# georgesterpu/avsr-tf1

Measured on AMD Instinct MI355X. Metric: utterances/sec (train step) at B=64 T_a=500 T_v=75, higher is better.
Workload: dtype f32; 1 GPU; c4: AV dual-attention (bimodal) video 1x256 + audio 3x256 uni-LSTM, scaled_luong, B=64 T_a=500x80 T_v=75 L=40; utterances_per_gpu=64, global_batch=64, T_a=500, F_a=80, T_v=75, F_v=128, T_dec=40, parallelism=dp1, video_frontend=resnet_cnn, launch=hipgraph, dropout=True

## Files before the change

### avsr-tf1_amd/csrc/rnn_persist.hip

```cpp
#include "step.h"
#include "avsr_hip.h"
#include "prof.h"
#include "persist.h"

#define P_MAX_TASKS 8
#define P_MAXC 8

namespace avsr {

struct PTask {
  const float* wt; const float* bias; const int* len;
  float* gates; float* cs;
  float* out; long out_sb, out_st;
  float* hs_w; long hs_sb, hs_st;
  const float* hs_r; long hsr_sb, hsr_st;
  const float* x_r; long x_sb, x_st;
  float* xt_w; long xt_sb, xt_st;
  float* h_final; float* c_final;
  int* done; const int* done_lower;
  int B, T, H, in, hoisted, reverse, nct, nct_lower, wg_begin, nrt, uw, part, prio;
  const int32_t* seed; float k_st, k_out, k_in; uint32_t r_st, r_out, r_in; int in_W, in_coff;
};
struct PLaunch { int ntask, wpx, ngroups, b0, npart, pwg[2]; int* err; int* claim; PTask task[P_MAX_TASKS]; };

__device__ __forceinline__ bool wait_ge2(const int* c0, int n0, const int* c1, int n1, int* err) {
  for (int spins = 0; spins < (1 << 21); ++spins) {
    const int a = c0 ? __hip_atomic_load(c0, __ATOMIC_RELAXED, __HIP_MEMORY_SCOPE_AGENT) : n0;
    const int b = c1 ? __hip_atomic_load(c1, __ATOMIC_RELAXED, __HIP_MEMORY_SCOPE_AGENT) : n1;
    if (a >= n0 && b >= n1) return true;
    if ((spins & 1023) == 1023 && __hip_atomic_load(err, __ATOMIC_RELAXED, __HIP_MEMORY_SCOPE_AGENT)) return false;
    __builtin_amdgcn_s_sleep(1);
  }
  __hip_atomic_store(err, 1, __ATOMIC_RELAXED, __HIP_MEMORY_SCOPE_AGENT);
  return false;
}

#ifdef PERSIST_TIMING
#define TICK(k) { const long now_ = __builtin_amdgcn_s_memtime(); tm[k] += now_ - last_; last_ = now_; }
#else
#define TICK(k)
#endif
#define P_XC 4
#define P_HC 4

__global__ __launch_bounds__(256) void rnn_persist_fwd_kernel(const PLaunch L) {
  __shared__ __attribute__((aligned(16))) float red[4][2][16][16];
  int ti = 0;
#pragma unroll
  for (int i = 1; i < P_MAX_TASKS; ++i)
    if (i < L.ntask && (int)blockIdx.x >= L.task[i].wg_begin) ti = i;
  ti = __builtin_amdgcn_readfirstlane(ti);
  const PTask& tk = L.task[ti];
  const int local = blockIdx.x - tk.wg_begin;
  const int rt = local / tk.nct, ct = local % tk.nct;
  const int row0 = rt * 16, col0 = ct * 32, unit0 = ct * 8;
  const int tid = threadIdx.x, lane = tid & 63, wave = tid >> 6;
  const int i = lane & 15, q = lane >> 4;
  const int H = tk.H, T = tk.T;
  const int hoisted = tk.hoisted, reverse = tk.reverse;
  const int Kx = hoisted ? 0 : tk.in;
  const int ncx = (Kx + 15) >> 4, nchh = (H + 15) >> 4;
  const int xg0 = (wave * ncx) / 4, nxw = ((wave + 1) * ncx) / 4 - xg0;
  const int hg0 = (wave * nchh) / 4, nhw = ((wave + 1) * nchh) / 4 - hg0;
  const long ldw = tk.in + H;

  f32x4 wx[P_XC][2], wh[P_HC][2];
#pragma unroll
  for (int nt = 0; nt < 2; ++nt) {
    const int col = col0 + nt * 16 + i;
#pragma unroll
    for (int c = 0; c < P_XC; ++c) {
      const int k = (xg0 + c) * 16 + 4 * q;
      wx[c][nt] = (c < nxw && col < 4 * H && k < Kx) ? ld4(tk.wt + (long)col * ldw + k) : f32x4{0.f, 0.f, 0.f, 0.f};
    }
#pragma unroll
    for (int c = 0; c < P_HC; ++c) {
      const int k = (hg0 + c) * 16 + 4 * q;
      wh[c][nt] = (c < nhw && col < 4 * H && k < H) ? ld4(tk.wt + (long)col * ldw + tk.in + k) : f32x4{0.f, 0.f, 0.f, 0.f};
    }
  }

  const int er = tid >> 3, eu = tid & 7;
  const int b = row0 + er, u = unit0 + eu;
  const bool eok = tid < 128 && b < tk.B && u < H;
  const int len_b = eok ? (tk.len ? tk.len[b] : T) : 0;
  f32x4 bias4 = {0.f, 0.f, 0.f, 0.f};
  if (eok && tk.bias) bias4 = ld4(tk.bias + u * 4);
  float c_state = 0.f, h_state = 0.f;

  const int ab = row0 + i;
  const bool aok = ab < tk.B;
  const int len_a = aok ? (tk.len ? tk.len[ab] : T) : 0;
  const int xrow = (int)(ab * tk.x_sb) + 4 * q, hrow = (int)(ab * tk.hsr_sb) + 4 * q;
  const int x_st = (int)tk.x_st, h_st = (int)tk.hsr_st;
  const float* const x_r = tk.x_r; const float* const hs_r = tk.hs_r;
  const int nct = tk.nct, nct_lower = tk.nct_lower;
  int* const done_mine = tk.done + (long)rt * T;
  const int* const done_low = hoisted ? nullptr : tk.done_lower + (long)rt * T;
  const int rec_b = b * T * H + u;
  const int out_b = (int)(b * tk.out_sb) + u, hsw_b = (int)(b * tk.hs_sb) + u, xtw_b = (int)(b * tk.xt_sb) + u;
  const int out_st = (int)tk.out_st, hs_st = (int)tk.hs_st, xt_st = (int)tk.xt_st;
  float* const gates_p = tk.gates; float* const cs_p = tk.cs; float* const out_p = tk.out;
  float* const hsw_p = tk.hs_w; float* const xtw_p = tk.xt_w;
  const bool drop_on = tk.seed != nullptr;
  const uint32_t seedv = drop_on ? (uint32_t)tk.seed[0] : 0u;
  const float k_st = tk.k_st, k_out = tk.k_out, k_in = tk.k_in;
  const uint32_t r_st = tk.r_st, r_out = tk.r_out, r_in = tk.r_in;
  const int in_W = tk.in_W, in_coff = tk.in_coff;

  f32x4 xcur[P_XC];
#pragma unroll
  for (int c = 0; c < P_XC; ++c) xcur[c] = f32x4{0.f, 0.f, 0.f, 0.f};
  auto load_x = [&](int t, f32x4* dst) {
    const bool v = aok && t < len_a;
    const int xo = xrow + (reverse ? len_a - 1 - t : t) * x_st;
#pragma unroll
    for (int c = 0; c < P_XC; ++c) {
      const int k = (xg0 + c) * 16;
      dst[c] = (c < nxw && v && k + 4 * q < Kx) ? ld4_sc1(x_r + (xo + k)) : f32x4{0.f, 0.f, 0.f, 0.f};
    }
  };
  if (done_low) {
    if (tid == 0) wait_ge2(done_low, nct_lower, nullptr, 0, L.err);
    __syncthreads();
    load_x(0, xcur);
  }

  f32x4 znext = {0.f, 0.f, 0.f, 0.f};
  if (eok && hoisted && 0 < len_b) znext = ld4(gates_p + (long)(rec_b + (reverse ? len_b - 1 : 0) * H) * 4);
#ifdef PERSIST_TIMING
  long tm[6] = {0, 0, 0, 0, 0, 0};
#endif
  for (int t = 0; t < T; ++t) {
#ifdef PERSIST_TIMING
    long last_ = __builtin_amdgcn_s_memtime();
#endif
    f32x4 zpre = znext;
    asm volatile("" : "+v"(zpre));
    if (tid == 0) {
      const int tl = t + 1 < T ? t + 1 : T - 1;
      wait_ge2(t > 0 ? done_mine + (t - 1) : nullptr, nct, done_low ? done_low + tl : nullptr, nct_lower, L.err);
    }
    lds_barrier();
    TICK(0)

    const bool avalid = aok && t < len_a;
    const int ho_ = hrow + (reverse ? len_a - 1 - t : t) * h_st;
    f32x4 hv[P_HC];
#pragma unroll
    for (int c = 0; c < P_HC; ++c) {
      const int k = (hg0 + c) * 16;
      hv[c] = (c < nhw && avalid && t > 0 && k + 4 * q < H) ? ld4_sc1(hs_r + (ho_ + k)) : f32x4{0.f, 0.f, 0.f, 0.f};
    }
    f32x4 acc[2][2];
#pragma unroll
    for (int nt = 0; nt < 2; ++nt)
#pragma unroll
      for (int e = 0; e < 2; ++e) acc[nt][e] = f32x4{0.f, 0.f, 0.f, 0.f};
#pragma unroll
    for (int c = 0; c < P_XC; ++c)
      if (c < nxw) {
#pragma unroll
        for (int nt = 0; nt < 2; ++nt)
#pragma unroll
          for (int e = 0; e < 4; ++e)
            acc[nt][e & 1] = __builtin_amdgcn_mfma_f32_16x16x4f32(xcur[c][e], wx[c][nt][e], acc[nt][e & 1], 0, 0, 0);
      }
    if (done_low && t + 1 < T) load_x(t + 1, xcur);
    if (eok && hoisted && t + 1 < len_b) znext = ld4(gates_p + (long)(rec_b + (reverse ? len_b - 2 - t : t + 1) * H) * 4);
    asm volatile("" ::: "memory");
#ifdef PERSIST_TIMING
    asm volatile("s_waitcnt vmcnt(0)" ::: "memory");
    TICK(1)
#endif
#pragma unroll
    for (int c = 0; c < P_HC; ++c)
      if (c < nhw) {
#pragma unroll
        for (int nt = 0; nt < 2; ++nt)
#pragma unroll
          for (int e = 0; e < 4; ++e)
            acc[nt][e & 1] = __builtin_amdgcn_mfma_f32_16x16x4f32(hv[c][e], wh[c][nt][e], acc[nt][e & 1], 0, 0, 0);
      }
#pragma unroll
    for (int nt = 0; nt < 2; ++nt) {
      const f32x4 s4 = acc[nt][0] + acc[nt][1];
#pragma unroll
      for (int r = 0; r < 4; ++r) red[wave][nt][(lane >> 4) * 4 + r][lane & 15] = s4[r];
    }
    lds_barrier();
    TICK(2)

    if (eok) {
      const bool valid = t < len_b;
      if (valid) {
        const int tau = reverse ? len_b - 1 - t : t;
        const long bt = (long)b * T + tau;
        f32x4 z = bias4 + zpre;
#pragma unroll
        for (int g = 0; g < 4; ++g) {
          const int cc = eu * 4 + g;
          z[g] += red[0][cc >> 4][er][cc & 15] + red[1][cc >> 4][er][cc & 15] + red[2][cc >> 4][er][cc & 15] + red[3][cc >> 4][er][cc & 15];
        }
        f32x4 g4;
        g4[0] = p_sigmoid(z[0]); g4[1] = p_tanh(z[1]); g4[2] = p_sigmoid(z[2] + 1.0f); g4[3] = p_sigmoid(z[3]);
        float c = g4[2] * c_state + g4[0] * g4[1];
        c = fminf(1.0f, fmaxf(-1.0f, c));
        const float h = g4[3] * p_tanh(c);
        const uint32_t oidx = (uint32_t)(bt * H + u);
        const float ho = h * p_drop(drop_on, seedv, r_out, oidx, k_out);
        const float hs = h * p_drop(drop_on, seedv, r_st, oidx, k_st);
        st_sc1(out_p + (out_b + tau * out_st), ho);
        if (hsw_p) st_sc1(hsw_p + (hsw_b + tau * hs_st), hs);
        if (xtw_p) st_sc1(xtw_p + (xtw_b + tau * xt_st), ho * p_drop(drop_on, seedv, r_in, (uint32_t)(bt * in_W + in_coff + u), k_in));
        st4(gates_p + (long)(rec_b + tau * H) * 4, g4);
        cs_p[rec_b + tau * H] = c;
        c_state = c;
        h_state = hs;
      } else {
        st_sc1(out_p + (out_b + t * out_st), 0.f);
        if (hsw_p) st_sc1(hsw_p + (hsw_b + t * hs_st), 0.f);
        if (xtw_p) st_sc1(xtw_p + (xtw_b + t * xt_st), 0.f);
      }
    }
    TICK(3)
    asm volatile("s_waitcnt vmcnt(0)" ::: "memory");
    __syncthreads();
    TICK(4)
    if (tid == 0) __hip_atomic_fetch_add(done_mine + t, 1, __ATOMIC_RELAXED, __HIP_MEMORY_SCOPE_AGENT);
    TICK(5)
  }
#ifdef PERSIST_TIMING
  if (tid == 0 && local == 0)
    for (int k = 0; k < 6; ++k) L.err[16 + ti * 8 + k] = (int)(tm[k] / T);
#endif
  if (eok) {
    if (tk.h_final) tk.h_final[(long)b * H + u] = h_state;
    if (tk.c_final) tk.c_final[(long)b * H + u] = c_state;
  }
}


template <int R, bool Q4 = false>
__global__ __launch_bounds__(256) __attribute__((amdgpu_waves_per_eu(3, 3))) void rnn_persist_fwd_xcd_kernel(const PLaunch L) {
  static_assert(!Q4 || R == 8, "4x4 recurrent product: 8-row groups");
  __shared__ __attribute__((aligned(16))) float red[4][4][R][16];
  __shared__ __attribute__((aligned(16))) float red4[Q4 ? 2048 : 4];
  __shared__ int s_slot;
  const int gx = __builtin_amdgcn_readfirstlane(xcc_id());
  if (threadIdx.x == 0) s_slot = __hip_atomic_fetch_add(L.claim + gx, 1, __ATOMIC_RELAXED, __HIP_MEMORY_SCOPE_AGENT);
  __syncthreads();
  const int slot = __builtin_amdgcn_readfirstlane(s_slot);
  const int tid = threadIdx.x, lane = tid & 63, wave = tid >> 6;
  const int part = L.npart == 2 ? gx >> 2 : 0;
  const int g = L.npart == 2 ? gx & 3 : gx;
  if (g >= L.ngroups || slot >= (L.npart == 2 ? L.pwg[part] : L.wpx)) return;
  int ti = -1;
#pragma unroll
  for (int i = 0; i < P_MAX_TASKS; ++i)
    if (i < L.ntask && L.task[i].part == part && slot >= L.task[i].wg_begin) ti = i;
  ti = __builtin_amdgcn_readfirstlane(ti);
  if (ti < 0) return;
  const PTask& tk = L.task[ti];
  if (tk.prio == 3) __builtin_amdgcn_s_setprio(3);
  else if (tk.prio == 2) __builtin_amdgcn_s_setprio(2);
  else if (tk.prio == 1) __builtin_amdgcn_s_setprio(1);
  const int ct = slot - tk.wg_begin;
  const int UW = tk.uw, uw_shift = UW == 16 ? 4 : 3;
  const int row0 = L.b0 + g * R, col0 = ct * UW * 4, unit0 = ct * UW;
  const int i = lane & 15, q = lane >> 4;
  const int H = tk.H, T = tk.T;
  const int hoisted = tk.hoisted, reverse = tk.reverse;
  const bool wide = hoisted && UW == 16;
  const int Kx = hoisted ? 0 : tk.in;
  const int ncx = (Kx + 15) >> 4, nchh = (H + 15) >> 4;
  const int xg0 = (wave * ncx) / 4, nxw = ((wave + 1) * ncx) / 4 - xg0;
  const int hg0 = (wave * nchh) / 4, nhw = ((wave + 1) * nchh) / 4 - hg0;
  const long ldw = tk.in + H;

  f32x4 wa[P_XC][2], wb[P_HC][2];
  f32x4 wq[Q4 ? 16 : 1];
  const int q4_col = (hoisted && UW == 16) ? lane : (lane & 31);
  const int q4_kb = hg0 * 16 + ((hoisted && UW == 16) ? 0 : 32 * (lane >> 5));
  if constexpr (Q4) {
    const int col = col0 + q4_col;
#pragma unroll
    for (int ab = 0; ab < 16; ++ab) {
      f32x4 v = {0.f, 0.f, 0.f, 0.f};
      if (ab < ((hoisted && UW == 16) ? 16 : 8) && col < 4 * H) v = ld4(tk.wt + (long)col * ldw + tk.in + q4_kb + 4 * ab);
      wq[ab] = v;
    }
  }
#pragma unroll
  for (int nt = 0; nt < 2; ++nt) {
    const int col = col0 + nt * 16 + i;
#pragma unroll
    for (int c = 0; c < P_HC; ++c) {
      const int k = (hg0 + c) * 16 + 4 * q;
      wb[c][nt] = (!Q4 && c < nhw && col < 4 * H && k < H) ? ld4(tk.wt + (long)col * ldw + tk.in + k) : f32x4{0.f, 0.f, 0.f, 0.f};
    }
#pragma unroll
    for (int c = 0; c < P_XC; ++c) {
      f32x4 v = {0.f, 0.f, 0.f, 0.f};
      if (wide) {
        const int k = (hg0 + c) * 16 + 4 * q, col2 = col + 32;
        if (!Q4 && c < nhw && col2 < 4 * H && k < H) v = ld4(tk.wt + (long)col2 * ldw + tk.in + k);
      } else {
        const int k = (xg0 + c) * 16 + 4 * q;
        if (c < nxw && col < 4 * H && k < Kx) v = ld4(tk.wt + (long)col * ldw + k);
      }
      wa[c][nt] = v;
    }
  }

  if constexpr (Q4) {
    if (!wide) {
#pragma unroll
      for (int c = 0; c < P_XC; ++c)
#pragma unroll
        for (int nt = 0; nt < 2; ++nt) wq[8 + 2 * c + nt] = wa[c][nt];
    }
  }
  const int er = tid >> uw_shift, eu = tid & (UW - 1);
  const int b = row0 + er, u = unit0 + eu;
  const bool eok = tid < R * UW && b < tk.B && u < H;
  const int len_b = eok ? (tk.len ? tk.len[b] : T) : 0;
  f32x4 bias4 = {0.f, 0.f, 0.f, 0.f};
  if (eok && tk.bias) bias4 = ld4(tk.bias + u * 4);
  float c_state = 0.f, h_state = 0.f;

  constexpr bool PT = (R == 8);
  const int sub = PT ? (i >> 3) : 0;
  const int ab = row0 + (PT ? (i & 7) : i);
  const bool aok = (PT || i < R) && ab < tk.B;
  const int len_a = aok ? (tk.len ? tk.len[ab] : T) : 0;
  const int xrow = (int)(ab * tk.x_sb) + 4 * q, hrow = (int)(ab * tk.hsr_sb) + 4 * q;
  const int q4_r0 = row0 + (lane & 3), q4_r1 = q4_r0 + 4;
  const int q4a_k = hg0 * 16 + 4 * (lane >> 2);
  const int q4_len0 = (Q4 && q4_r0 < tk.B) ? (tk.len ? tk.len[q4_r0] : T) : 0, q4_len1 = (Q4 && q4_r1 < tk.B) ? (tk.len ? tk.len[q4_r1] : T) : 0;
  const int q4_h0 = (int)(q4_r0 * tk.hsr_sb) + q4a_k, q4_h1 = (int)(q4_r1 * tk.hsr_sb) + q4a_k;
  const int x_st = (int)tk.x_st, h_st = (int)tk.hsr_st;
  const __amdgpu_buffer_rsrc_t x_rs = make_rsrc(tk.x_r), h_rs = make_rsrc(tk.hs_r), z_rs = make_rsrc(tk.gates);
  const bool has_low = !hoisted;
  int* const my_flag = tk.done + gx * 32 + ct;
  const int* poll_ptr = nullptr;
  if (wave == 0) {
    if (lane < 32) { if (lane < tk.nct) poll_ptr = tk.done + gx * 32 + lane; }
    else if (has_low && lane - 32 < tk.nct_lower) poll_ptr = tk.done_lower + gx * 32 + (lane - 32);
  }
  const int rec_b = b * T * H + u;
  const int out_b = (int)(b * tk.out_sb) + u, hsw_b = (int)(b * tk.hs_sb) + u, xtw_b = (int)(b * tk.xt_sb) + u;
  const int out_st = (int)tk.out_st, hs_st = (int)tk.hs_st, xt_st = (int)tk.xt_st;
  float* const gates_p = tk.gates; float* const cs_p = tk.cs; float* const out_p = tk.out;
  float* const hsw_p = tk.hs_w; float* const xtw_p = tk.xt_w;
  const bool drop_on = tk.seed != nullptr;
  const uint32_t seedv = drop_on ? (uint32_t)tk.seed[0] : 0u;
  const float k_st = tk.k_st, k_out = tk.k_out, k_in = tk.k_in;
  const uint32_t r_st = tk.r_st, r_out = tk.r_out, r_in = tk.r_in;
  const int in_W = tk.in_W, in_coff = tk.in_coff;

  auto wait_progress = [&](int need_own, int need_low) {
    if (wave != 0) return;
    const int need = lane < 32 ? need_own : need_low;
    for (int spins = 0; spins < (1 << 21); ++spins) {
      const int v = poll_ptr ? __hip_atomic_load(poll_ptr, __ATOMIC_RELAXED, __HIP_MEMORY_SCOPE_AGENT) : 0x7fffffff;
      if (__all(v >= need)) return;
      if ((spins & 1023) == 1023 && __hip_atomic_load(L.err, __ATOMIC_RELAXED, __HIP_MEMORY_SCOPE_AGENT)) return;
    }
    if (lane == 0) __hip_atomic_store(L.err, 1, __ATOMIC_RELAXED, __HIP_MEMORY_SCOPE_AGENT);
  };

  f32x4 xcur[P_XC];
#pragma unroll
  for (int c = 0; c < P_XC; ++c) xcur[c] = f32x4{0.f, 0.f, 0.f, 0.f};
  auto load_x = [&](int t0, f32x4* dst) {
    const int t = t0 + sub;
    const bool v = aok && t < len_a;
    const int xo = xrow + (reverse ? len_a - 1 - t : t) * x_st;
#pragma unroll
    for (int c = 0; c < P_XC; ++c) {
      const int k = (xg0 + c) * 16;
      dst[c] = ldb_sc1(x_rs, (c < nxw && v && k + 4 * q < Kx) ? (xo + k) * 4 : P_OOB);
    }
  };
  if (has_low) {
    wait_progress(0, PT ? (2 < T ? 2 : T) : 1);
    __syncthreads();
    load_x(0, xcur);
  }
  f32x4 accx[2] = {f32x4{0.f, 0.f, 0.f, 0.f}, f32x4{0.f, 0.f, 0.f, 0.f}};
  f32x4 znext = {0.f, 0.f, 0.f, 0.f};
  znext = ldb4(z_rs, (eok && hoisted && 0 < len_b) ? (rec_b + (reverse ? len_b - 1 : 0) * H) * 16 : P_OOB);
#ifdef PERSIST_TIMING
  long tm[6] = {0, 0, 0, 0, 0, 0};
#endif
  for (int t = 0; t < T; ++t) {
#ifdef PERSIST_TIMING
    long last_ = __builtin_amdgcn_s_memtime();
#endif
    f32x4 zpre = znext;
    asm volatile("" : "+v"(zpre));
    wait_progress(t, PT ? ((t & 1) ? (t + 3 < T ? t + 3 : T) : 0) : (t + 2 < T ? t + 2 : T));
    lds_barrier();
    TICK(0)
    const bool avalid = aok && t < len_a && (!PT || sub == (t & 1));
    const int ho_ = hrow + (reverse ? len_a - 1 - t : t) * h_st;
    f32x4 hv[P_HC];
    f32x4 a_lo = {0.f, 0.f, 0.f, 0.f}, a_hi = {0.f, 0.f, 0.f, 0.f};
    if constexpr (Q4) {
      a_lo = ldb_sc1(h_rs, (t > 0 && t < q4_len0) ? (q4_h0 + (reverse ? q4_len0 - 1 - t : t) * h_st) * 4 : P_OOB);
      a_hi = ldb_sc1(h_rs, (t > 0 && t < q4_len1) ? (q4_h1 + (reverse ? q4_len1 - 1 - t : t) * h_st) * 4 : P_OOB);
    } else {
#pragma unroll
      for (int c = 0; c < P_HC; ++c) {
        const int k = (hg0 + c) * 16;
        hv[c] = ldb_sc1(h_rs, (c < nhw && avalid && t > 0 && k + 4 * q < H) ? (ho_ + k) * 4 : P_OOB);
      }
    }
#ifdef PERSIST_TIMING
    asm volatile("s_waitcnt vmcnt(0)" ::: "memory");
    TICK(1)
#endif
    f32x4 acc[4];
#pragma unroll
    for (int nt = 0; nt < 4; ++nt) acc[nt] = f32x4{0.f, 0.f, 0.f, 0.f};
    if (!hoisted) {
      if (!PT || !(t & 1)) {
#pragma unroll
        for (int c = 0; c < P_XC; ++c)
          if (c < nxw) {
#pragma unroll
            for (int nt = 0; nt < 2; ++nt)
#pragma unroll
              for (int e = 0; e < 4; ++e)
                acc[nt] = __builtin_amdgcn_mfma_f32_16x16x4f32(xcur[c][e], Q4 ? wq[Q4 ? 8 + 2 * c + nt : 0][e] : wa[c][nt][e], acc[nt], 0, 0, 0);
          }
        if (PT) { accx[0] = acc[0]; accx[1] = acc[1]; }
      } else {
        acc[0] = accx[0]; acc[1] = accx[1];
      }
      if (!PT) load_x(t + 1 < T ? t + 1 : T, xcur);
      else if (t & 1) load_x(t + 1 < T ? t + 1 : T, xcur);
    }
    znext = ldb4(z_rs, (eok && hoisted && t + 1 < len_b) ? (rec_b + (reverse ? len_b - 2 - t : t + 1) * H) * 16 : P_OOB);
    asm volatile("" ::: "memory");
    if constexpr (Q4) {
      f32x4 r0 = {0.f, 0.f, 0.f, 0.f}, r1 = r0;
#define Q4_STEP(CB, AB)                                                                                   \
      _Pragma("unroll") for (int v = 0; v < 4; ++v) {                                                     \
        r0 = __builtin_amdgcn_mfma_f32_4x4x1f32(a_lo[v], wq[AB][v], r0, CB, AB, 0);                       \
        r1 = __builtin_amdgcn_mfma_f32_4x4x1f32(a_hi[v], wq[AB][v], r1, CB, AB, 0);                       \
      }
      if (wide) {
        Q4_STEP(4, 0) Q4_STEP(4, 1) Q4_STEP(4, 2) Q4_STEP(4, 3) Q4_STEP(4, 4) Q4_STEP(4, 5) Q4_STEP(4, 6) Q4_STEP(4, 7)
        Q4_STEP(4, 8) Q4_STEP(4, 9) Q4_STEP(4, 10) Q4_STEP(4, 11) Q4_STEP(4, 12) Q4_STEP(4, 13) Q4_STEP(4, 14) Q4_STEP(4, 15)
      } else {
        Q4_STEP(3, 0) Q4_STEP(3, 1) Q4_STEP(3, 2) Q4_STEP(3, 3) Q4_STEP(3, 4) Q4_STEP(3, 5) Q4_STEP(3, 6) Q4_STEP(3, 7)
      }
#undef Q4_STEP
      float* const dst = wide ? red4 + (wave * 8) * 64 + q4_col : red4 + ((wave * 2 + (lane >> 5)) * 8) * 32 + q4_col;
      const int rs = wide ? 64 : 32;
#pragma unroll
      for (int r = 0; r < 4; ++r) { dst[r * rs] = r0[r]; dst[(4 + r) * rs] = r1[r]; }
    } else {
#pragma unroll
    for (int c = 0; c < P_HC; ++c)
      if (c < nhw) {
#pragma unroll
        for (int nt = 0; nt < 2; ++nt)
#pragma unroll
          for (int e = 0; e < 4; ++e)
            acc[nt] = __builtin_amdgcn_mfma_f32_16x16x4f32(hv[c][e], wb[c][nt][e], acc[nt], 0, 0, 0);
        if (wide) {
#pragma unroll
          for (int nt = 0; nt < 2; ++nt)
#pragma unroll
            for (int e = 0; e < 4; ++e)
              acc[2 + nt] = __builtin_amdgcn_mfma_f32_16x16x4f32(hv[c][e], wa[c][nt][e], acc[2 + nt], 0, 0, 0);
        }
      }
    }
    if (PT ? (q >> 1) == (t & 1) : q < R / 4) {
      const int rq = PT ? (q & 1) : q;
#pragma unroll
      for (int nt = 0; nt < 4; ++nt)
#pragma unroll
        for (int r = 0; r < 4; ++r) red[wave][nt][rq * 4 + r][i] = acc[nt][r];
    }
    lds_barrier();
    TICK(2)
    __builtin_amdgcn_s_setprio(3);
    if (eok) {
      const bool valid = t < len_b;
      if (valid) {
        const int tau = reverse ? len_b - 1 - t : t;
        const long bt = (long)b * T + tau;
        f32x4 z = bias4 + zpre;
        {
          const int c0 = eu * 4;
          if constexpr (Q4) {
            f32x4 s4 = {0.f, 0.f, 0.f, 0.f};
            if (UW == 16) {
#pragma unroll
              for (int w = 0; w < 4; ++w) s4 += *reinterpret_cast<const f32x4*>(&red4[(w * 8 + er) * 64 + c0]);
            } else {
#pragma unroll
              for (int w = 0; w < 8; ++w) s4 += *reinterpret_cast<const f32x4*>(&red4[(w * 8 + er) * 32 + c0]);
              const int ct4 = c0 >> 4, cl = c0 & 15;
              s4 += (*reinterpret_cast<const f32x4*>(&red[0][ct4][er][cl]) + *reinterpret_cast<const f32x4*>(&red[1][ct4][er][cl])) +
                    (*reinterpret_cast<const f32x4*>(&red[2][ct4][er][cl]) + *reinterpret_cast<const f32x4*>(&red[3][ct4][er][cl]));
            }
            z += s4;
          } else {
            const int ct4 = c0 >> 4, cl = c0 & 15;
            z += (*reinterpret_cast<const f32x4*>(&red[0][ct4][er][cl]) + *reinterpret_cast<const f32x4*>(&red[1][ct4][er][cl])) +
                 (*reinterpret_cast<const f32x4*>(&red[2][ct4][er][cl]) + *reinterpret_cast<const f32x4*>(&red[3][ct4][er][cl]));
          }
        }
        f32x4 g4;
        g4[0] = p_sigmoid(z[0]); g4[1] = p_tanh(z[1]); g4[2] = p_sigmoid(z[2] + 1.0f); g4[3] = p_sigmoid(z[3]);
        float c = g4[2] * c_state + g4[0] * g4[1];
        c = fminf(1.0f, fmaxf(-1.0f, c));
        const float h = g4[3] * p_tanh(c);
        const uint32_t oidx = (uint32_t)(bt * H + u);
        const float ho = h * p_drop(drop_on, seedv, r_out, oidx, k_out);
        const float hs = h * p_drop(drop_on, seedv, r_st, oidx, k_st);
        out_p[out_b + tau * out_st] = ho;
        if (hsw_p) hsw_p[hsw_b + tau * hs_st] = hs;
        if (xtw_p) xtw_p[xtw_b + tau * xt_st] = ho * p_drop(drop_on, seedv, r_in, (uint32_t)(bt * in_W + in_coff + u), k_in);
        st4(gates_p + (long)(rec_b + tau * H) * 4, g4);
        cs_p[rec_b + tau * H] = c;
        c_state = c;
        h_state = hs;
      } else {
        out_p[out_b + t * out_st] = 0.f;
        if (hsw_p) hsw_p[hsw_b + t * hs_st] = 0.f;
        if (xtw_p) xtw_p[xtw_b + t * xt_st] = 0.f;
      }
    }
    TICK(3)
    if (tk.prio == 3) __builtin_amdgcn_s_setprio(3);
    else if (tk.prio == 2) __builtin_amdgcn_s_setprio(2);
    else if (tk.prio == 1) __builtin_amdgcn_s_setprio(1);
    else __builtin_amdgcn_s_setprio(0);
    asm volatile("s_waitcnt vmcnt(0)" ::: "memory");
    __syncthreads();
    TICK(4)
    if (tid == 0) __hip_atomic_store(my_flag, t + 1, __ATOMIC_RELAXED, __HIP_MEMORY_SCOPE_WORKGROUP);
    TICK(5)
  }
#ifdef PERSIST_TIMING
  if (tid == 0 && ct == 0 && g == 0)
    for (int k = 0; k < 6; ++k) L.err[16 + ti * 8 + k] = (int)(tm[k] / T);
#endif
  if (eok) {
    if (tk.h_final) tk.h_final[(long)b * H + u] = h_state;
    if (tk.c_final) tk.c_final[(long)b * H + u] = c_state;
  }
}

int32_t* g_sync = nullptr;
int g_persist_mode = 3;

int64_t g_sync_ints = 0;

}

extern "C" int avsr_rnn_set_persistent(int32_t* sync, int64_t ints) {
  avsr::g_sync = sync; avsr::g_sync_ints = sync ? ints : 0;
  return AVSR_OK;
}

namespace avsr {

static double g_fwd_flops = 0.0;
static int build_tasks(const avsr_rnn_stack* st, int n, bool local, int32_t* sync, int64_t sync_ints, PLaunch& L, int* wg_out, long* words_out,
                       bool parts = false) {
  L = PLaunch{};
  g_fwd_flops = 0.0;
  if (parts && (!local || n != 2 || st[0].B > 64)) return AVSR_ERR_UNSUPPORTED;
  int wg = 0;
  long ctr = P_HDR + 8;
  for (int i = 0; i < n; ++i) {
    const avsr_rnn_stack& S = st[i];
    if (S.cell != 0 || S.B != st[0].B) return AVSR_ERR_UNSUPPORTED;
    const int nrt = local ? (S.B + 7) / 8 : (S.B + 15) / 16;
    if (parts) { if (i == 1) L.pwg[0] = wg; wg = 0; }
    for (int l = 0; l < S.n_layers; ++l) {
      const avsr_rnn_layer& Ly = S.layer[l];
      if (L.ntask >= P_MAX_TASKS) return AVSR_ERR_UNSUPPORTED;
      const int H = Ly.units, in = Ly.in_dim;
      if ((long)S.B * (S.T + 2) * (Ly.ld_out > 4 * H ? Ly.ld_out : 4 * H) >= (1L << 29)) return AVSR_ERR_UNSUPPORTED;
      if (H % 8 || !Ly.out || H > 64 * P_HC || (!Ly.hoisted && in > 64 * P_XC) || in % 4) return AVSR_ERR_UNSUPPORTED;
      if (!Ly.hoisted && l == 0) return AVSR_ERR_UNSUPPORTED;
      if (S.seed && !Ly.hs_seq) return AVSR_ERR_UNSUPPORTED;
      PTask& tk = L.task[L.ntask++];
      tk.wt = Ly.wt; tk.bias = Ly.bias; tk.len = S.len;
      tk.gates = Ly.gates; tk.cs = Ly.cs;
      tk.out = Ly.out + Ly.ld_out + Ly.out_col; tk.out_sb = (long)(S.T + 2) * Ly.ld_out; tk.out_st = Ly.ld_out;
      const float* hseq; long hld;
      if (S.seed) { tk.hs_w = Ly.hs_seq + H; tk.hs_sb = (long)(S.T + 2) * H; tk.hs_st = H; hseq = Ly.hs_seq; hld = H; }
      else { hseq = Ly.out + Ly.out_col; hld = Ly.ld_out; }
      tk.hs_r = hseq + (S.reverse ? 2 * hld : 0); tk.hsr_sb = (long)(S.T + 2) * hld; tk.hsr_st = hld;
      if (!Ly.hoisted) {
        const avsr_rnn_layer& Lo = S.layer[l - 1];
        if (S.seed) { if (!Lo.xt_seq) return AVSR_ERR_UNSUPPORTED; tk.x_r = Lo.xt_seq + Lo.units; tk.x_sb = (long)(S.T + 2) * Lo.units; tk.x_st = Lo.units; }
        else { tk.x_r = Lo.out + Lo.ld_out + Lo.out_col; tk.x_sb = (long)(S.T + 2) * Lo.ld_out; tk.x_st = Lo.ld_out; }
      }
      if (S.seed && Ly.xt_seq) { tk.xt_w = Ly.xt_seq + H; tk.xt_sb = (long)(S.T + 2) * H; tk.xt_st = H; }
      tk.h_final = Ly.h_final; tk.c_final = Ly.c_final;
      tk.B = S.B; tk.T = S.T; tk.H = H; tk.in = in; tk.hoisted = Ly.hoisted; tk.reverse = S.reverse;
      g_fwd_flops += 2.0 * S.B * S.T * ((Ly.hoisted ? 0 : in) + H) * 4.0 * H;
      tk.uw = (local && Ly.hoisted && H % 16 == 0) ? 16 : 8;
      tk.prio = Ly.hoisted ? 0 : 2;
      tk.nct = H / tk.uw; tk.nrt = nrt; tk.wg_begin = wg; tk.part = parts ? i : 0;
      if (tk.nct > 32) return AVSR_ERR_UNSUPPORTED;
      wg += local ? tk.nct : nrt * tk.nct;
      tk.done = sync + ctr;
      ctr += local ? 8 * 32 : (long)nrt * S.T;
      if (!Ly.hoisted) { tk.done_lower = L.task[L.ntask - 2].done; tk.nct_lower = L.task[L.ntask - 2].nct; }
      if (S.seed) {
        const uint32_t cid = (uint32_t)(S.cell_id_base + l);
        tk.seed = S.seed; tk.k_st = S.keep_state; tk.k_out = S.keep_out; tk.k_in = 1.0f;
        tk.r_st = cid * 4 + 1; tk.r_out = cid * 4 + 2;
        if (l + 1 < S.n_layers) { tk.k_in = S.keep_in; tk.r_in = (cid + 1) * 4; tk.in_W = H; tk.in_coff = 0; }
        else if (S.consumer_width > 0) { tk.k_in = S.consumer_keep; tk.r_in = (uint32_t)S.consumer_stream; tk.in_W = S.consumer_width; tk.in_coff = 0; }
      }
    }
  }
  if (ctr > sync_ints) return AVSR_ERR_UNSUPPORTED;
  if (parts) {
    L.pwg[1] = wg; L.npart = 2;
    if (L.pwg[0] > 96 || L.pwg[1] > 96) return AVSR_ERR_UNSUPPORTED;
    wg = L.pwg[0] > L.pwg[1] ? L.pwg[0] : L.pwg[1];
  }
  if (local ? wg > 96 : wg > 512) return AVSR_ERR_UNSUPPORTED;
  L.err = sync; L.claim = sync + P_HDR; L.wpx = wg; L.ngroups = 0; L.b0 = 0;
  *wg_out = wg; *words_out = ctr;
  return AVSR_OK;
}

}

extern "C" int avsr_rnn_set_persistent_mode(int mode) { avsr::g_persist_mode = mode; return AVSR_OK; }

int avsr_rnn_fwd_persistent(const avsr_rnn_stack* st, int32_t n, void* stream, int dry) {
  using namespace avsr;
  int32_t* sync = g_sync; const int64_t sync_ints = g_sync_ints;
  if (!sync) return AVSR_ERR_UNSUPPORTED;
  static thread_local PLaunch L;
  hipStream_t s = (hipStream_t)stream;
  int wg = 0; long words = 0;
  if ((g_persist_mode & 2) && build_tasks(st, n, true, sync, sync_ints, L, &wg, &words) == AVSR_OK) {
    if (dry) return AVSR_OK;
    const int B = st[0].B;
    const int R = B > 64 ? 16 : 8;
    for (int b0 = 0; b0 < B; b0 += 8 * R) {
      const int rows = B - b0 < 8 * R ? B - b0 : 8 * R;
      L.b0 = b0; L.ngroups = (rows + R - 1) / R;
      if (avsr::dev_zero(sync + P_HDR, sizeof(int32_t) * (words - P_HDR), s) != hipSuccess) return AVSR_ERR_HIP;
      {
        ProfScope ps(PROF_RNN_PERSIST_FWD, s, g_fwd_flops * rows / B);
        bool q4 = R == 8;
        for (int i = 0; i < L.ntask && q4; ++i) q4 = L.task[i].H == 256 && (L.task[i].hoisted ? L.task[i].uw == 16 : (L.task[i].uw == 8 && L.task[i].in == 256));
        if (R == 16) hipLaunchKernelGGL(rnn_persist_fwd_xcd_kernel<16>, dim3(8 * wg), dim3(256), 0, s, L);
        else if (q4) hipLaunchKernelGGL((rnn_persist_fwd_xcd_kernel<8, true>), dim3(8 * wg), dim3(256), 0, s, L);
        else hipLaunchKernelGGL(rnn_persist_fwd_xcd_kernel<8>, dim3(8 * wg), dim3(256), 0, s, L);
      }
      AVSR_CHECK_LAUNCH();
    }
    return AVSR_OK;
  }
  if ((g_persist_mode & 2) && build_tasks(st, n, true, sync, sync_ints, L, &wg, &words, true) == AVSR_OK) {
    if (dry) return AVSR_OK;
    const int B = st[0].B;
    L.b0 = 0; L.ngroups = (B + 15) / 16;
    if (avsr::dev_zero(sync + P_HDR, sizeof(int32_t) * (words - P_HDR), s) != hipSuccess) return AVSR_ERR_HIP;
    {
      ProfScope ps(PROF_RNN_PERSIST_FWD, s, g_fwd_flops);
      hipLaunchKernelGGL(rnn_persist_fwd_xcd_kernel<16>, dim3(8 * wg), dim3(256), 0, s, L);
    }
    AVSR_CHECK_LAUNCH();
    return AVSR_OK;
  }
  if ((g_persist_mode & 1) && build_tasks(st, n, false, sync, sync_ints, L, &wg, &words) == AVSR_OK) {
    if (dry) return AVSR_OK;
    if (avsr::dev_zero(sync + P_HDR, sizeof(int32_t) * (words - P_HDR), s) != hipSuccess) return AVSR_ERR_HIP;
    {
      ProfScope ps(PROF_RNN_PERSIST_FWD, s, g_fwd_flops);
      hipLaunchKernelGGL(rnn_persist_fwd_kernel, dim3(wg), dim3(256), 0, s, L);
    }
    AVSR_CHECK_LAUNCH();
    return AVSR_OK;
  }
  return AVSR_ERR_UNSUPPORTED;
}
```

Before: 5735 utterances/sec.

## Add helper workgroups that compute upper-layer input projections ahead of recurrence

Adds 'help' tasks to the persistent LSTM forward kernel. Dedicated workgroups compute the input-to-gate product for non-hoisted upper layers and write it to the gates buffer step by step. The recurrent cell task then reads these precomputed gates as a hoisted layer, behind a new progress flag. This takes the input matmul off the critical recurrent path and lets it overlap with the lower layer. In exchange it needs more workgroups, another cross-workgroup sync counter and changed priorities, and the path is only taken when a mode bit is set.

Result: slower. 5671 utterances/sec (-1.1%).

```diff
diff --git a/avsr-tf1_amd/csrc/rnn_persist.hip b/avsr-tf1_amd/csrc/rnn_persist.hip
--- a/avsr-tf1_amd/csrc/rnn_persist.hip
+++ b/avsr-tf1_amd/csrc/rnn_persist.hip
@@ -19,6 +19,7 @@
   float* h_final; float* c_final;
   int* done; const int* done_lower;
   int B, T, H, in, hoisted, reverse, nct, nct_lower, wg_begin, nrt, uw, part, prio;
+  int kind, fed;
   const int32_t* seed; float k_st, k_out, k_in; uint32_t r_st, r_out, r_in; int in_W, in_coff;
 };
 struct PLaunch { int ntask, wpx, ngroups, b0, npart, pwg[2]; int* err; int* claim; PTask task[P_MAX_TASKS]; };
@@ -241,8 +242,115 @@
 }
 
 
-template <int R, bool Q4 = false>
+__device__ __forceinline__ void fwd_help_task(const PLaunch& L, const PTask& tk, int ti, int gx, int g, int ct, float (*red)[2][16][16]) {
+  const int tid = threadIdx.x, lane = tid & 63, wave = tid >> 6;
+  const int i = lane & 15, q = lane >> 4;
+  const int H = tk.H, T = tk.T, Kx = tk.in, reverse = tk.reverse;
+  const int row0 = L.b0 + g * 8, col0 = ct * 64, unit0 = ct * 16;
+  const int ncx = (Kx + 15) >> 4;
+  const int xg0 = (wave * ncx) / 4, nxw = ((wave + 1) * ncx) / 4 - xg0;
+  const long ldw = tk.in + H;
+  f32x4 w[P_XC][4];
+#pragma unroll
+  for (int c = 0; c < P_XC; ++c)
+#pragma unroll
+    for (int nt = 0; nt < 4; ++nt) {
+      const int col = col0 + nt * 16 + i, k = (xg0 + c) * 16 + 4 * q;
+      w[c][nt] = (c < nxw && col < 4 * H && k < Kx) ? ld4(tk.wt + (long)col * ldw + k) : f32x4{0.f, 0.f, 0.f, 0.f};
+    }
+  const int sub = i >> 3, ab = row0 + (i & 7);
+  const bool aok = ab < tk.B;
+  const int len_a = aok ? (tk.len ? tk.len[ab] : T) : 0;
+  const int xrow = (int)(ab * tk.x_sb) + 4 * q, x_st = (int)tk.x_st;
+  const __amdgpu_buffer_rsrc_t x_rs = make_rsrc(tk.x_r);
+  const int er = tid >> 4, eu = tid & 15, esub = er >> 3;
+  const int eb = row0 + (er & 7), u = unit0 + eu;
+  const bool eok = eb < tk.B && u < H;
+  const int len_e = eok ? (tk.len ? tk.len[eb] : T) : 0;
+  const int rec_b = eb * T * H + u;
+  float* const gates_p = tk.gates;
+  int* const my_flag = tk.done + gx * 32 + ct;
+  const int* const poll_ptr = (wave == 0 && lane < tk.nct_lower) ? tk.done_lower + gx * 32 + lane : nullptr;
+#ifdef PERSIST_TIMING
+  long tm[6] = {0, 0, 0, 0, 0, 0};
+#endif
+  for (int t0 = 0; t0 < T; t0 += 2) {
+#ifdef PERSIST_TIMING
+    long last_ = __builtin_amdgcn_s_memtime();
+#endif
+    const int upto = t0 + 2 < T ? t0 + 2 : T;
+    if (wave == 0) {
+      bool ok = false;
+      for (int spins = 0; spins < (1 << 21) && !ok; ++spins) {
+        const int v = poll_ptr ? __hip_atomic_load(poll_ptr, __ATOMIC_RELAXED, __HIP_MEMORY_SCOPE_AGENT) : 0x7fffffff;
+        ok = __all(v >= upto) || ((spins & 1023) == 1023 && __hip_atomic_load(L.err, __ATOMIC_RELAXED, __HIP_MEMORY_SCOPE_AGENT));
+      }
+      if (!ok && lane == 0) __hip_atomic_store(L.err, 1, __ATOMIC_RELAXED, __HIP_MEMORY_SCOPE_AGENT);
+    }
+    lds_barrier();
+    TICK(0)
+    const int t = t0 + sub;
+    const bool v = aok && t < len_a;
+    const int xo = xrow + (reverse ? len_a - 1 - t : t) * x_st;
+    f32x4 xv[P_XC];
+#pragma unroll
+    for (int c = 0; c < P_XC; ++c) {
+      const int k = (xg0 + c) * 16;
+      xv[c] = ldb_sc1(x_rs, (c < nxw && v && k + 4 * q < Kx) ? (xo + k) * 4 : P_OOB);
+    }
+#ifdef PERSIST_TIMING
+    asm volatile("s_waitcnt vmcnt(0)" ::: "memory");
+    TICK(1)
+#endif
+    f32x4 acc[4];
+#pragma unroll
+    for (int nt = 0; nt < 4; ++nt) acc[nt] = f32x4{0.f, 0.f, 0.f, 0.f};
+#pragma unroll
+    for (int c = 0; c < P_XC; ++c)
+      if (c < nxw) {
+#pragma unroll
+        for (int e = 0; e < 4; ++e)
+#pragma unroll
+          for (int nt = 0; nt < 4; ++nt)
+            acc[nt] = __builtin_amdgcn_mfma_f32_16x16x4f32(xv[c][e], w[c][nt][e], acc[nt], 0, 0, 0);
+          __builtin_amdgcn_sched_barrier(0);
+          __builtin_amdgcn_s_sleep(2);
+          __builtin_amdgcn_sched_barrier(0);
+      }
+    TICK(2)
+    const int te = t0 + esub;
+    const int tau = reverse ? len_e - 1 - te : te;
+#pragma unroll
+    for (int half = 0; half < 2; ++half) {
+      if (half) lds_barrier();
+#pragma unroll
+      for (int nt = 0; nt < 2; ++nt)
+#pragma unroll
+        for (int r = 0; r < 4; ++r) red[wave][nt][q * 4 + r][i] = acc[half * 2 + nt][r];
+      lds_barrier();
+      if ((eu >> 3) == half && eok && te < len_e) {
+        const int ct2 = (eu >> 2) & 1, cl = (eu & 3) * 4;
+        const f32x4 z = (*reinterpret_cast<const f32x4*>(&red[0][ct2][er][cl]) + *reinterpret_cast<const f32x4*>(&red[1][ct2][er][cl])) +
+                        (*reinterpret_cast<const f32x4*>(&red[2][ct2][er][cl]) + *reinterpret_cast<const f32x4*>(&red[3][ct2][er][cl]));
+        st4(gates_p + (long)(rec_b + tau * H) * 4, z);
+      }
+    }
+    TICK(3)
+    asm volatile("s_waitcnt vmcnt(0)" ::: "memory");
+    __syncthreads();
+    TICK(4)
+    if (tid == 0) __hip_atomic_store(my_flag, upto, __ATOMIC_RELAXED, __HIP_MEMORY_SCOPE_WORKGROUP);
+    TICK(5)
+  }
+#ifdef PERSIST_TIMING
+  if (tid == 0 && ct == 0 && g == 0)
+    for (int k = 0; k < 6; ++k) L.err[16 + ti * 8 + k] = (int)(tm[k] / T);
+#endif
+}
+
+template <int R, bool Q4 = false, bool FED = false>
 __global__ __launch_bounds__(256) __attribute__((amdgpu_waves_per_eu(3, 3))) void rnn_persist_fwd_xcd_kernel(const PLaunch L) {
+  static_assert(!FED || R == 8, "HELP tasks: 8-row groups");
   static_assert(!Q4 || R == 8, "4x4 recurrent product: 8-row groups");
   __shared__ __attribute__((aligned(16))) float red[4][4][R][16];
   __shared__ __attribute__((aligned(16))) float red4[Q4 ? 2048 : 4];
@@ -266,6 +374,9 @@
   else if (tk.prio == 2) __builtin_amdgcn_s_setprio(2);
   else if (tk.prio == 1) __builtin_amdgcn_s_setprio(1);
   const int ct = slot - tk.wg_begin;
+  if constexpr (FED) {
+    if (tk.kind == 1) { fwd_help_task(L, tk, ti, gx, g, ct, reinterpret_cast<float (*)[2][16][16]>(&red[0][0][0][0])); return; }
+  }
   const int UW = tk.uw, uw_shift = UW == 16 ? 4 : 3;
   const int row0 = L.b0 + g * R, col0 = ct * UW * 4, unit0 = ct * UW;
   const int i = lane & 15, q = lane >> 4;
@@ -342,11 +453,12 @@
   const int x_st = (int)tk.x_st, h_st = (int)tk.hsr_st;
   const __amdgpu_buffer_rsrc_t x_rs = make_rsrc(tk.x_r), h_rs = make_rsrc(tk.hs_r), z_rs = make_rsrc(tk.gates);
   const bool has_low = !hoisted;
+  const bool fed = FED && tk.fed != 0;
   int* const my_flag = tk.done + gx * 32 + ct;
   const int* poll_ptr = nullptr;
   if (wave == 0) {
     if (lane < 32) { if (lane < tk.nct) poll_ptr = tk.done + gx * 32 + lane; }
-    else if (has_low && lane - 32 < tk.nct_lower) poll_ptr = tk.done_lower + gx * 32 + (lane - 32);
+    else if ((has_low || fed) && lane - 32 < tk.nct_lower) poll_ptr = tk.done_lower + gx * 32 + (lane - 32);
   }
   const int rec_b = b * T * H + u;
   const int out_b = (int)(b * tk.out_sb) + u, hsw_b = (int)(b * tk.hs_sb) + u, xtw_b = (int)(b * tk.xt_sb) + u;
@@ -390,7 +502,12 @@
   }
   f32x4 accx[2] = {f32x4{0.f, 0.f, 0.f, 0.f}, f32x4{0.f, 0.f, 0.f, 0.f}};
   f32x4 znext = {0.f, 0.f, 0.f, 0.f};
-  znext = ldb4(z_rs, (eok && hoisted && 0 < len_b) ? (rec_b + (reverse ? len_b - 1 : 0) * H) * 16 : P_OOB);
+  if (fed) {
+    wait_progress(0, 1);
+    __syncthreads();
+  }
+  auto ld_z = [&](int byte_off) { return FED ? ldb_sc1(z_rs, byte_off) : ldb4(z_rs, byte_off); };
+  znext = ld_z((eok && hoisted && 0 < len_b) ? (rec_b + (reverse ? len_b - 1 : 0) * H) * 16 : P_OOB);
 #ifdef PERSIST_TIMING
   long tm[6] = {0, 0, 0, 0, 0, 0};
 #endif
@@ -442,7 +559,7 @@
       if (!PT) load_x(t + 1 < T ? t + 1 : T, xcur);
       else if (t & 1) load_x(t + 1 < T ? t + 1 : T, xcur);
     }
-    znext = ldb4(z_rs, (eok && hoisted && t + 1 < len_b) ? (rec_b + (reverse ? len_b - 2 - t : t + 1) * H) * 16 : P_OOB);
+    znext = ld_z((eok && hoisted && t + 1 < len_b) ? (rec_b + (reverse ? len_b - 2 - t : t + 1) * H) * 16 : P_OOB);
     asm volatile("" ::: "memory");
     if constexpr (Q4) {
       f32x4 r0 = {0.f, 0.f, 0.f, 0.f}, r1 = r0;
@@ -575,9 +692,11 @@
 
 static double g_fwd_flops = 0.0;
 static int build_tasks(const avsr_rnn_stack* st, int n, bool local, int32_t* sync, int64_t sync_ints, PLaunch& L, int* wg_out, long* words_out,
-                       bool parts = false) {
+                       bool parts = false, int max_help = 0, int* nhelp_out = nullptr) {
   L = PLaunch{};
   g_fwd_flops = 0.0;
+  int nhelp = 0, help_cell[P_MAX_TASKS];
+  if (nhelp_out) *nhelp_out = 0;
   if (parts && (!local || n != 2 || st[0].B > 64)) return AVSR_ERR_UNSUPPORTED;
   int wg = 0;
   long ctr = P_HDR + 8;
@@ -594,6 +713,7 @@
       if (H % 8 || !Ly.out || H > 64 * P_HC || (!Ly.hoisted && in > 64 * P_XC) || in % 4) return AVSR_ERR_UNSUPPORTED;
       if (!Ly.hoisted && l == 0) return AVSR_ERR_UNSUPPORTED;
       if (S.seed && !Ly.hs_seq) return AVSR_ERR_UNSUPPORTED;
+      const bool fed = local && !parts && !Ly.hoisted && S.B <= 64 && H % 16 == 0 && nhelp < max_help;
       PTask& tk = L.task[L.ntask++];
       tk.wt = Ly.wt; tk.bias = Ly.bias; tk.len = S.len;
       tk.gates = Ly.gates; tk.cs = Ly.cs;
@@ -609,16 +729,17 @@
       }
       if (S.seed && Ly.xt_seq) { tk.xt_w = Ly.xt_seq + H; tk.xt_sb = (long)(S.T + 2) * H; tk.xt_st = H; }
       tk.h_final = Ly.h_final; tk.c_final = Ly.c_final;
-      tk.B = S.B; tk.T = S.T; tk.H = H; tk.in = in; tk.hoisted = Ly.hoisted; tk.reverse = S.reverse;
+      tk.B = S.B; tk.T = S.T; tk.H = H; tk.in = in; tk.hoisted = Ly.hoisted || fed; tk.reverse = S.reverse; tk.fed = fed;
       g_fwd_flops += 2.0 * S.B * S.T * ((Ly.hoisted ? 0 : in) + H) * 4.0 * H;
-      tk.uw = (local && Ly.hoisted && H % 16 == 0) ? 16 : 8;
-      tk.prio = Ly.hoisted ? 0 : 2;
+      tk.uw = (local && tk.hoisted && H % 16 == 0) ? 16 : 8;
+      tk.prio = tk.hoisted ? 0 : 2;
       tk.nct = H / tk.uw; tk.nrt = nrt; tk.wg_begin = wg; tk.part = parts ? i : 0;
       if (tk.nct > 32) return AVSR_ERR_UNSUPPORTED;
       wg += local ? tk.nct : nrt * tk.nct;
       tk.done = sync + ctr;
       ctr += local ? 8 * 32 : (long)nrt * S.T;
       if (!Ly.hoisted) { tk.done_lower = L.task[L.ntask - 2].done; tk.nct_lower = L.task[L.ntask - 2].nct; }
+      if (fed) help_cell[nhelp++] = L.ntask - 1;
       if (S.seed) {
         const uint32_t cid = (uint32_t)(S.cell_id_base + l);
         tk.seed = S.seed; tk.k_st = S.keep_state; tk.k_out = S.keep_out; tk.k_in = 1.0f;
@@ -627,6 +748,22 @@
         else if (S.consumer_width > 0) { tk.k_in = S.consumer_keep; tk.r_in = (uint32_t)S.consumer_stream; tk.in_W = S.consumer_width; tk.in_coff = 0; }
       }
     }
+  }
+  if (nhelp_out) *nhelp_out = nhelp;
+  if (nhelp > 0)
+    for (int i = 0; i < L.ntask; ++i)
+      if (L.task[i].hoisted) L.task[i].prio = 1;
+  for (int j = 0; j < nhelp; ++j) {
+    if (L.ntask >= P_MAX_TASKS) return AVSR_ERR_UNSUPPORTED;
+    PTask& ck = L.task[help_cell[j]];
+    PTask& hk = L.task[L.ntask++];
+    hk = ck;
+    hk.kind = 1; hk.fed = 0; hk.hoisted = 0; hk.prio = 0; hk.uw = 16; hk.nct = hk.H / 16; hk.wg_begin = wg;
+    hk.h_final = nullptr; hk.c_final = nullptr;
+    wg += hk.nct;
+    hk.done = sync + ctr;
+    ctr += 8 * 32;
+    ck.done_lower = hk.done; ck.nct_lower = hk.nct;
   }
   if (ctr > sync_ints) return AVSR_ERR_UNSUPPORTED;
   if (parts) {
@@ -651,7 +788,13 @@
   static thread_local PLaunch L;
   hipStream_t s = (hipStream_t)stream;
   int wg = 0; long words = 0;
-  if ((g_persist_mode & 2) && build_tasks(st, n, true, sync, sync_ints, L, &wg, &words) == AVSR_OK) {
+  int rc = AVSR_ERR_UNSUPPORTED, nh = 0;
+  if (g_persist_mode & 2)
+    for (int mh = (g_persist_mode & 8) ? P_MAX_TASKS : 0; mh >= 0; mh = nh - 1) {
+      rc = build_tasks(st, n, true, sync, sync_ints, L, &wg, &words, false, mh, &nh);
+      if (rc == AVSR_OK || nh == 0) break;
+    }
+  if (rc == AVSR_OK) {
     if (dry) return AVSR_OK;
     const int B = st[0].B;
     const int R = B > 64 ? 16 : 8;
@@ -662,8 +805,10 @@
       {
         ProfScope ps(PROF_RNN_PERSIST_FWD, s, g_fwd_flops * rows / B);
         bool q4 = R == 8;
-        for (int i = 0; i < L.ntask && q4; ++i) q4 = L.task[i].H == 256 && (L.task[i].hoisted ? L.task[i].uw == 16 : (L.task[i].uw == 8 && L.task[i].in == 256));
+        for (int i = 0; i < L.ntask && q4; ++i) q4 = L.task[i].H == 256 && (L.task[i].kind == 1 || L.task[i].hoisted ? L.task[i].uw == 16 : (L.task[i].uw == 8 && L.task[i].in == 256));
         if (R == 16) hipLaunchKernelGGL(rnn_persist_fwd_xcd_kernel<16>, dim3(8 * wg), dim3(256), 0, s, L);
+        else if (nh > 0 && q4) hipLaunchKernelGGL((rnn_persist_fwd_xcd_kernel<8, true, true>), dim3(8 * wg), dim3(256), 0, s, L);
+        else if (nh > 0) hipLaunchKernelGGL((rnn_persist_fwd_xcd_kernel<8, false, true>), dim3(8 * wg), dim3(256), 0, s, L);
         else if (q4) hipLaunchKernelGGL((rnn_persist_fwd_xcd_kernel<8, true>), dim3(8 * wg), dim3(256), 0, s, L);
         else hipLaunchKernelGGL(rnn_persist_fwd_xcd_kernel<8>, dim3(8 * wg), dim3(256), 0, s, L);
       }
```
